# suleka96/siddhi

Measured on AMD Instinct MI355X. Metric: input events/sec + % HBM peak, partitioned pattern query, 1/2/4/8 MI355X, higher is better.
Workload: dtype f64

## Files before the change

siddhi_amd/csrc/kernels/pass0_dev.h:

```cpp
#pragma once
#include <type_traits>

#include "fastpath_dev.h"

namespace sm {
namespace {

constexpr int kP0Block = 1024;
constexpr int kP0Waves = kP0Block / 64;
constexpr int kP0Items = 4;
constexpr int kP0Tile = kP0Block * kP0Items;
constexpr int kP0Seg = 4;
static_assert(kBins == kP0Block && kP0Waves == 16, "one digit per thread, 16 waves");

__device__ __forceinline__ uint32_t sm_udot2(uint32_t a, uint32_t b, uint32_t c) {
#if defined(__HIP_DEVICE_COMPILE__)
  typedef unsigned short u16x2 __attribute__((ext_vector_type(2)));
  return __builtin_amdgcn_udot2(__builtin_bit_cast(u16x2, a), __builtin_bit_cast(u16x2, b), c, false);
#else
  return c + (a & 0xffffu) * (b & 0xffffu) + (a >> 16) * (b >> 16);
#endif
}

__device__ __forceinline__ uint32_t p0_before(const uint4& r0, const uint4& r1, int w) {
  const uint32_t word[8] = {r0.x, r0.y, r0.z, r0.w, r1.x, r1.y, r1.z, r1.w};
  uint32_t s = 0;
#pragma unroll
  for (int i = 0; i < 8; ++i) {
    const uint32_t m = 2 * i + 1 < w ? 0xffffffffu : (2 * i < w ? 0x0000ffffu : 0u);
    s = sm_udot2(word[i] & m, 0x00010001u, s);
  }
  return s;
}

__device__ __forceinline__ void p0_store_fence(uint4 (&rec)[kP0Items]) {
#if defined(__HIP_DEVICE_COMPILE__)
#pragma unroll
  for (int k = 0; k < kP0Items; ++k)
    asm volatile("" : "+v"(rec[k].x), "+v"(rec[k].y), "+v"(rec[k].z), "+v"(rec[k].w) : : "memory");
#else
  (void)rec;
#endif
}

__device__ __forceinline__ int64_t p0_opaque(int64_t v) {
#if defined(__HIP_DEVICE_COMPILE__)
  asm volatile("" : "+s"(v));
#endif
  return v;
}

template <typename S, typename = void>
struct p0_time_order : std::false_type {};
template <typename S>
struct p0_time_order<S, std::void_t<decltype(S::kTimeOrder)>> : std::integral_constant<bool, S::kTimeOrder> {};

__device__ __forceinline__ uint32_t p0_lane_before(uint32_t v) {
#if defined(__HIP_DEVICE_COMPILE__)
  return (uint32_t)__builtin_amdgcn_update_dpp((int)v, (int)v, 0x138 , 0xf, 0xf, false);
#else
  return __shfl_up(v, 1, 64);
#endif
}

template <typename Src>
__global__ void __launch_bounds__(kP0Block) pass0_kernel(Src src, uint4* __restrict__ drec, int64_t n, int64_t per,
                                                          int G, const uint32_t* __restrict__ cnt,
                                                          const uint32_t* __restrict__ dbase) {
  __shared__ __attribute__((aligned(16))) uint4 xb[kP0Tile];
  __shared__ __attribute__((aligned(16))) uint16_t wc[kBins][kP0Waves];
  __shared__ uint32_t tstart[kBins + 1];
  __shared__ uint32_t run[kBins];
  __shared__ uint32_t cst[kBins];
  __shared__ __attribute__((aligned(16))) uint4 carry[kBins][kP0Seg - 1];
  __shared__ uint32_t lw[kP0Waves];
  __shared__ uint32_t tlast[kP0Waves + 1];
  __shared__ uint32_t tbad;
  constexpr bool kTO = p0_time_order<Src>::value;

  const int tid = threadIdx.x, lane = tid & 63, w = wave_index();
  const int64_t lo = (int64_t)blockIdx.x * per;
  int64_t len = n - lo;
  if (len > per) len = per;
  if (len < 0) len = 0;
  src.init();
  uint4* row = (uint4*)&wc[tid][0];
  {
    const uint32_t r0 = dbase[tid] + cnt[(int64_t)tid * G + blockIdx.x];
    run[tid] = r0;
    cst[tid] = r0;
    row[0] = make_uint4(0, 0, 0, 0);
    row[1] = make_uint4(0, 0, 0, 0);
  }
  if constexpr (kTO) {
    if (tid == 0) {
      tbad = 0u;
      tlast[kP0Waves] = (lo > 0 && len > 0) ? (uint32_t)(src.time_at(lo - 1) - src.time0()) : 0u;
    }
  }
  lds_barrier();
  int tpar = 0;
  typename Src::Raw raw[kP0Items];
  auto load_tile = [&](int64_t base) {
    const int64_t rem = lo + len - base;
    const int tn = rem < kP0Tile ? (int)rem : kP0Tile;
    base = p0_opaque(base);
#pragma unroll
    for (int k = 0; k < kP0Items; ++k) {
      const int e = w * 64 * kP0Items + k * 64 + lane;
      if (e < tn) raw[k] = src.load(base + e);
    }
  };
  const int64_t end = lo + len;
  if (len > 0) load_tile(lo);
  int ptile_n = 0;
  bool plast = false;
  uint4 cq0, cq1, cq2;
  static_assert(kP0Seg == 4, "three carried records at most");

  for (int64_t base = lo;; base += kP0Tile) {
    const bool more = base < end;
    const int tile_n = (int)((end - base) < kP0Tile ? (end - base) : kP0Tile);
    const bool last = base + kP0Tile >= end;
    uint4 rec[kP0Items];
#if defined(__HIP_DEVICE_COMPILE__)
    __builtin_amdgcn_s_waitcnt(0x0F70);
#endif
    uint32_t tfirst = 0;
    if (more) {
      uint32_t tq[kP0Items];
      bool tb = false;
#pragma unroll
      for (int k = 0; k < kP0Items; ++k) {
        const int e = w * 64 * kP0Items + k * 64 + lane;
        if constexpr (kTO) tq[k] = 0u;
        if (e < tile_n) {
          rec[k] = src.record(raw[k], base + e);
          if constexpr (kTO) {
            const int64_t rel = src.time_of(raw[k]) - src.time0();
            tq[k] = (uint32_t)rel;
            tb |= ((uint64_t)rel >> 32) != 0;
          }
        }
      }
      if constexpr (kTO) {
#pragma unroll
        for (int k = 0; k < kP0Items; ++k) {
          const int e = w * 64 * kP0Items + k * 64 + lane;
          uint32_t pv = p0_lane_before(tq[k]);
          const uint32_t pl = wave_read_lane(tq[k > 0 ? k - 1 : 0], 63);
          if (lane == 0) pv = k > 0 ? pl : tq[0];
          tb |= e < tile_n && tq[k] < pv;
        }
        if (lane == 63) tlast[w < kP0Waves - 1 ? w : kP0Waves - 1 + tpar] = tq[kP0Items - 1];
        if (tb) tbad = 1u;
        tfirst = tq[0];
      }
    }
    p0_store_fence(rec);

    if (base != lo) {
      const uint32_t rn = run[tid], c0 = cst[tid], ct = tstart[tid + 1] - tstart[tid];
      const uint32_t lim = plast ? 0xffffffffu : ((rn + ct) & ~(uint32_t)(kP0Seg - 1));
      const uint32_t nfl = (rn != c0 && (plast || lim > c0)) ? rn - c0 : 0u;
      if (nfl > 0) drec[c0] = cq0;
      if (nfl > 1) drec[c0 + 1] = cq1;
      if (nfl > 2) drec[c0 + 2] = cq2;
#pragma unroll
      for (int r = 0; r < kP0Items; ++r) {
        const int s = r * kP0Block + tid;
        if (s < ptile_n) {
          const uint4 x = xb[s];
          const uint32_t d = x.x & (kBins - 1);
          const uint32_t rd = run[d], td = tstart[d];
          const uint32_t dest = rd + (uint32_t)s - td;
          const uint32_t ld = plast ? 0xffffffffu : ((rd + tstart[d + 1] - td) & ~(uint32_t)(kP0Seg - 1));
          if (dest < ld) {
            drec[dest] = x;
          } else {
            const uint32_t cd = cst[d];
            carry[d][dest - (cd > ld ? cd : ld)] = x;
          }
        }
      }
      lds_barrier();
      run[tid] = rn + ct;
      if (lim != 0xffffffffu && lim > c0) cst[tid] = lim;
    }
    if (!more) break;

    uint32_t dg[kP0Items], lp = 0;
    static_assert(kP0Items * 64 <= 256 && kP0Items <= 4, "a record's rank within (wave, digit) fits 8 bits");
#pragma unroll
    for (int k = 0; k < kP0Items; ++k) {
      const int e = w * 64 * kP0Items + k * 64 + lane;
      const bool valid = e < tile_n;
      dg[k] = valid ? rec[k].x & (kBins - 1) : 0u;
      const uint64_t peers = peer_mask(dg[k], valid);
      uint32_t old = 0;
      if (valid) old = wc[dg[k]][w];
      wave_lockstep();
      const uint32_t below = lanes_below(peers);
      if (valid && below == 0) wc[dg[k]][w] = (uint16_t)(old + (uint32_t)__popcll(peers));
      wave_lockstep();
      lp |= (old + below) << (8 * k);
    }
    if (!last) load_tile(base + kP0Tile);
    lds_barrier();
    if constexpr (kTO) {
      if (lane == 0 && w * 64 * kP0Items < tile_n && tfirst < tlast[w > 0 ? w - 1 : kP0Waves - 1 + (tpar ^ 1)])
        tbad = 1u;
      tpar ^= 1;
    }

    uint32_t ct = 0;
    {
      const uint4 r0 = row[0], r1 = row[1];
      const uint32_t word[8] = {r0.x, r0.y, r0.z, r0.w, r1.x, r1.y, r1.z, r1.w};
#pragma unroll
      for (int i = 0; i < 8; ++i) ct = sm_udot2(word[i], 0x00010001u, ct);
      uint32_t tot;
      tstart[tid] = block_excl<kP0Block>(ct, lw, &tot);
      if (tid == 0) tstart[kBins] = tot;
    }
    const uint32_t rn = run[tid], c0 = cst[tid];
    const uint32_t lim = last ? 0xffffffffu : ((rn + ct) & ~(uint32_t)(kP0Seg - 1));
    lds_barrier();

#pragma unroll
    for (int k = 0; k < kP0Items; ++k) {
      const int e = w * 64 * kP0Items + k * 64 + lane;
      if (e < tile_n) {
        const uint32_t d = rec[k].x & (kBins - 1);
        const uint4* rr = (const uint4*)&wc[d][0];
        xb[tstart[d] + p0_before(rr[0], rr[1], w) + ((lp >> (8 * k)) & 0xffu)] = rec[k];
      }
    }
    const uint32_t nfl = (rn != c0 && (last || lim > c0)) ? rn - c0 : 0u;
    if (nfl > 0) cq0 = carry[tid][0];
    if (nfl > 1) cq1 = carry[tid][1];
    if (nfl > 2) cq2 = carry[tid][2];
    lds_barrier();
    row[0] = make_uint4(0, 0, 0, 0);
    row[1] = make_uint4(0, 0, 0, 0);
    ptile_n = tile_n;
    plast = last;
  }
  src.flush();
  if constexpr (kTO) {
    if (tid == 0 && tbad != 0u) src.time_bad();
  }
}

}
}
```

Baseline: 30.65 billion.

## Precompute per-wave digit offsets in LDS and keep run count in registers

The per-(digit, wave) count table is split into two halves. After the block scan, each thread writes per-wave exclusive prefix offsets, including the tile start, back into that table. The scatter then reads one uint16 offset instead of two uint4 rows plus an 8-step masked dot-product sum. Per-digit dest offsets and limits are also precomputed into doff/dlim, and the running count moves from LDS to a register, cutting LDS reads and arithmetic in the hot scatter and flush loops. The risk is that the 16-bit packed offsets could overflow if tile offsets exceed 65535, though the tile size of 4096 keeps them in range.

New measurement: 30.94 billion (median of 6 runs). No clear change (+1.0%).

```diff
diff --git a/siddhi_amd/csrc/kernels/pass0_dev.h b/siddhi_amd/csrc/kernels/pass0_dev.h
--- a/siddhi_amd/csrc/kernels/pass0_dev.h
+++ b/siddhi_amd/csrc/kernels/pass0_dev.h
@@ -22,17 +22,6 @@
 #endif
 }
 
-__device__ __forceinline__ uint32_t p0_before(const uint4& r0, const uint4& r1, int w) {
-  const uint32_t word[8] = {r0.x, r0.y, r0.z, r0.w, r1.x, r1.y, r1.z, r1.w};
-  uint32_t s = 0;
-#pragma unroll
-  for (int i = 0; i < 8; ++i) {
-    const uint32_t m = 2 * i + 1 < w ? 0xffffffffu : (2 * i < w ? 0x0000ffffu : 0u);
-    s = sm_udot2(word[i] & m, 0x00010001u, s);
-  }
-  return s;
-}
-
 __device__ __forceinline__ void p0_store_fence(uint4 (&rec)[kP0Items]) {
 #if defined(__HIP_DEVICE_COMPILE__)
 #pragma unroll
@@ -68,9 +57,9 @@
                                                           int G, const uint32_t* __restrict__ cnt,
                                                           const uint32_t* __restrict__ dbase) {
   __shared__ __attribute__((aligned(16))) uint4 xb[kP0Tile];
-  __shared__ __attribute__((aligned(16))) uint16_t wc[kBins][kP0Waves];
-  __shared__ uint32_t tstart[kBins + 1];
-  __shared__ uint32_t run[kBins];
+  __shared__ __attribute__((aligned(16))) uint16_t wc[2][kBins][kP0Waves / 2];
+  __shared__ uint32_t doff[kBins];
+  __shared__ uint32_t dlim[kBins];
   __shared__ uint32_t cst[kBins];
   __shared__ __attribute__((aligned(16))) uint4 carry[kBins][kP0Seg - 1];
   __shared__ uint32_t lw[kP0Waves];
@@ -84,13 +73,15 @@
   if (len > per) len = per;
   if (len < 0) len = 0;
   src.init();
-  uint4* row = (uint4*)&wc[tid][0];
+  uint4* const row0 = (uint4*)&wc[0][tid][0];
+  uint4* const row1 = (uint4*)&wc[1][tid][0];
+  uint16_t(*const wcw)[kP0Waves / 2] = wc[w >> 3];
+  const int wq = w & 7;
+  uint32_t run = dbase[tid] + cnt[(int64_t)tid * G + blockIdx.x], pct = 0;
   {
-    const uint32_t r0 = dbase[tid] + cnt[(int64_t)tid * G + blockIdx.x];
-    run[tid] = r0;
-    cst[tid] = r0;
-    row[0] = make_uint4(0, 0, 0, 0);
-    row[1] = make_uint4(0, 0, 0, 0);
+    cst[tid] = run;
+    *row0 = make_uint4(0, 0, 0, 0);
+    *row1 = make_uint4(0, 0, 0, 0);
   }
   if constexpr (kTO) {
     if (tid == 0) {
@@ -114,7 +105,6 @@
   const int64_t end = lo + len;
   if (len > 0) load_tile(lo);
   int ptile_n = 0;
-  bool plast = false;
   uint4 cq0, cq1, cq2;
   static_assert(kP0Seg == 4, "three carried records at most");
 
@@ -160,9 +150,8 @@
     p0_store_fence(rec);
 
     if (base != lo) {
-      const uint32_t rn = run[tid], c0 = cst[tid], ct = tstart[tid + 1] - tstart[tid];
-      const uint32_t lim = plast ? 0xffffffffu : ((rn + ct) & ~(uint32_t)(kP0Seg - 1));
-      const uint32_t nfl = (rn != c0 && (plast || lim > c0)) ? rn - c0 : 0u;
+      const uint32_t rn = run, c0 = cst[tid], lim = dlim[tid];
+      const uint32_t nfl = (rn != c0 && lim > c0) ? rn - c0 : 0u;
       if (nfl > 0) drec[c0] = cq0;
       if (nfl > 1) drec[c0 + 1] = cq1;
       if (nfl > 2) drec[c0 + 2] = cq2;
@@ -172,9 +161,7 @@
         if (s < ptile_n) {
           const uint4 x = xb[s];
           const uint32_t d = x.x & (kBins - 1);
-          const uint32_t rd = run[d], td = tstart[d];
-          const uint32_t dest = rd + (uint32_t)s - td;
-          const uint32_t ld = plast ? 0xffffffffu : ((rd + tstart[d + 1] - td) & ~(uint32_t)(kP0Seg - 1));
+          const uint32_t dest = doff[d] + (uint32_t)s, ld = dlim[d];
           if (dest < ld) {
             drec[dest] = x;
           } else {
@@ -184,7 +171,7 @@
         }
       }
       lds_barrier();
-      run[tid] = rn + ct;
+      run = rn + pct;
       if (lim != 0xffffffffu && lim > c0) cst[tid] = lim;
     }
     if (!more) break;
@@ -198,10 +185,10 @@
       dg[k] = valid ? rec[k].x & (kBins - 1) : 0u;
       const uint64_t peers = peer_mask(dg[k], valid);
       uint32_t old = 0;
-      if (valid) old = wc[dg[k]][w];
+      if (valid) old = wcw[dg[k]][wq];
       wave_lockstep();
       const uint32_t below = lanes_below(peers);
-      if (valid && below == 0) wc[dg[k]][w] = (uint16_t)(old + (uint32_t)__popcll(peers));
+      if (valid && below == 0) wcw[dg[k]][wq] = (uint16_t)(old + (uint32_t)__popcll(peers));
       wave_lockstep();
       lp |= (old + below) << (8 * k);
     }
@@ -214,17 +201,27 @@
     }
 
     uint32_t ct = 0;
+    const uint32_t rn = run, c0 = cst[tid];
+    uint32_t lim;
     {
-      const uint4 r0 = row[0], r1 = row[1];
+      const uint4 r0 = *row0, r1 = *row1;
       const uint32_t word[8] = {r0.x, r0.y, r0.z, r0.w, r1.x, r1.y, r1.z, r1.w};
 #pragma unroll
       for (int i = 0; i < 8; ++i) ct = sm_udot2(word[i], 0x00010001u, ct);
       uint32_t tot;
-      tstart[tid] = block_excl<kP0Block>(ct, lw, &tot);
-      if (tid == 0) tstart[kBins] = tot;
-    }
-    const uint32_t rn = run[tid], c0 = cst[tid];
-    const uint32_t lim = last ? 0xffffffffu : ((rn + ct) & ~(uint32_t)(kP0Seg - 1));
+      const uint32_t ts = block_excl<kP0Block>(ct, lw, &tot);
+      lim = last ? 0xffffffffu : ((rn + ct) & ~(uint32_t)(kP0Seg - 1));
+      doff[tid] = rn - ts;
+      dlim[tid] = lim;
+      uint32_t acc = ts, b[8];
+#pragma unroll
+      for (int i = 0; i < 8; ++i) {
+        b[i] = acc * 0x00010001u + (word[i] << 16);
+        acc = sm_udot2(word[i], 0x00010001u, acc);
+      }
+      *row0 = make_uint4(b[0], b[1], b[2], b[3]);
+      *row1 = make_uint4(b[4], b[5], b[6], b[7]);
+    }
     lds_barrier();
 
 #pragma unroll
@@ -232,19 +229,18 @@
       const int e = w * 64 * kP0Items + k * 64 + lane;
       if (e < tile_n) {
         const uint32_t d = rec[k].x & (kBins - 1);
-        const uint4* rr = (const uint4*)&wc[d][0];
-        xb[tstart[d] + p0_before(rr[0], rr[1], w) + ((lp >> (8 * k)) & 0xffu)] = rec[k];
-      }
-    }
-    const uint32_t nfl = (rn != c0 && (last || lim > c0)) ? rn - c0 : 0u;
+        xb[(uint32_t)wcw[d][wq] + ((lp >> (8 * k)) & 0xffu)] = rec[k];
+      }
+    }
+    const uint32_t nfl = (rn != c0 && lim > c0) ? rn - c0 : 0u;
     if (nfl > 0) cq0 = carry[tid][0];
     if (nfl > 1) cq1 = carry[tid][1];
     if (nfl > 2) cq2 = carry[tid][2];
     lds_barrier();
-    row[0] = make_uint4(0, 0, 0, 0);
-    row[1] = make_uint4(0, 0, 0, 0);
+    *row0 = make_uint4(0, 0, 0, 0);
+    *row1 = make_uint4(0, 0, 0, 0);
     ptile_n = tile_n;
-    plast = last;
+    pct = ct;
   }
   src.flush();
   if constexpr (kTO) {
```
